# yahoo0742/COSNet

Measured on AMD Instinct MI355X. Metric: frame-pairs/sec (fwd+bwd) at 473x473 RGBD, higher is better.
Workload: dtype bf16; 1 GPU; RGBDSegmentation_RAA train step (fwd+loss+bwd+SGD), 473x473, batch 4 pairs/GPU; model=RGBDSegmentation_RAA(Bottleneck,[3,4,23,3],[3,4,6,3],1), global_batch=4, parallelism=dp1

## Files before the change

cosnet_amd/_native.py:

```python
import ctypes
import os

import torch

_HERE = os.path.dirname(os.path.abspath(__file__))
LIB_PATH = os.environ.get("COSNET_HIP_LIB") or os.path.join(_HERE, "_lib", "libcosnet_hip.so")

DT_F32 = 0
DT_BF16 = 1

_P = ctypes.c_void_p
_I = ctypes.c_int
_L = ctypes.c_longlong
_F = ctypes.c_float
_S = ctypes.c_size_t

_SIGS = {
    "cn_conv_fwd": (_I, [_I, _P, _L, _I, _I, _I, _I, _P, _I, _I, _I, _I, _I, _I, _P, _P, _L, _I, _I, _P]),
    "cn_conv_fwd_ws": (_I, [_I, _P, _L, _I, _I, _I, _I, _P, _I, _I, _I, _I, _I, _I, _P, _P, _L, _I, _I,
                            _P, _S, _P]),
    "cn_conv_fwd_workspace_floats": (_S, [_I, _I, _I, _I]),
    "cn_conv_dgrad": (_I, [_I, _P, _L, _I, _I, _I, _I, _P, _I, _I, _I, _I, _I, _I, _P, _L, _I, _I, _I, _P]),
    "cn_conv_wgrad_workspace_floats": (_S, [_I, _I, _I, _I, _I, _I, _I, _I]),
    "cn_conv_wgrad": (_I, [_I, _P, _L, _I, _I, _I, _I, _P, _L, _I, _I, _I, _I, _I, _I, _I, _I, _P, _P, _P]),
# ... 31 lines not shown
                             _P, _L, _P, _L, _P, _P]),
    "cn_bn_apply_ex": (_I, [_I, _P, _L, _I, _I, _I, _P, _P, _P, _P, _P, _L, _P, _L, _P, _P, _P, _P, _I, _P,
                            _P, _L, _P, _L, _P, _P, _L, _P]),
    "cn_bn_apply_q8": (_I, [_I, _P, _L, _I, _I, _I, _P, _P, _P, _P, _P, _L, _P, _L, _P, _P, _P, _P, _I, _P,
                            _P, _L, _P, _L, _P, _P]),
    "cn_fp8_quant_static": (_I, [_I, _I, _P, _L, _I, _I, _P, _L, _P, _P]),
    "cn_bcast_rows_u8": (_I, [_P, _I, _I, _I, _P, _L, _P]),
    "cn_bn_set_tuning": (_I, [_I, _I]),
    "cn_bn_bwd": (_I, [_I, _P, _L, _P, _L, _P, _L, _I, _I, _P, _P, _P, _P, _I, _P, _P, _P, _P, _P, _L, _P, _L, _P, _P]),
    "cn_coatt_workspace_floats": (_S, [_I, _I, _I]),
    "cn_coatt_softmax": (_I, [_I, _P, _I, _I, _I, _P, _P, _P, _P]),
    "cn_coatt_dscore": (_I, [_I, _P, _P, _P, _P, _P, _P, _I, _I, _I, _P, _P]),
    "cn_coatt_fused_fwd": (_I, [_P, _L, _P, _L, _P, _L, _I, _I, _I, _P, _P, _L, _P]),
    "cn_coatt_fused_fwd_ws": (_I, [_P, _L, _P, _L, _P, _L, _I, _I, _I, _P, _P, _L, _P, _S, _P]),
    "cn_coatt_fused_workspace_bytes": (_S, [_I, _I, _I]),
    "cn_coatt_fused_fwd_idx": (_I, [_P, _L, _P, _L, _P, _L, _P, _P, _I, _I, _I, _P, _P, _L, _P, _S, _P]),
    "cn_gate_cat_idx": (_I, [_I, _P, _L, _P, _L, _P, _I, _I, _I, _P, _P, _P, _L, _P]),
    "cn_mean_groups": (_I, [_P, _I, _I, _I, _P, _P]),
    "cn_coatt_f8_workspace_bytes": (_S, [_I, _I]),
    "cn_coatt_f8_fwd": (_I, [_P, _L, _P, _L, _P, _L, _I, _I, _I, _P, _P, _L, _P, _P, _P, _S, _P]),
    "cn_coatt_f8_train_workspace_bytes": (_S, [_I, _I]),
    "cn_coatt_f8_train_fwd": (_I, [_P, _L, _P, _L, _P, _L, _I, _I, _I, _P, _P, _L, _P, _P, _P, _P, _P, _L, _P, _S, _P]),
    "cn_coatt_f8_bank_bytes": (_S, [_I, _I]),
    "cn_coatt_f8_bank_build": (_I, [_P, _L, _P, _L, _I, _I, _I, _P, _S, _P]),
    "cn_coatt_f8_fwd_idx": (_I, [_P, _P, _I, _P, _P, _I, _I, _I, _P, _P, _L, _P]),
    "cn_coatt_flash_fwd": (_I, [_P, _L, _P, _L, _P, _L, _I, _I, _I, _P, _P, _L, _P, _P, _P]),
    "cn_coatt_flash_fwd_ws": (_I, [_P, _L, _P, _L, _P, _L, _I, _I, _I, _P, _P, _L, _P, _P, _P, _S, _P]),
    "cn_coatt_flash_pv": (_I, [_P, _L, _P, _L, _P, _L, _P, _I, _I, _I, _P, _L, _I, _P]),
    "cn_coatt_flash_dvat": (_I, [_P, _L, _P, _L, _P, _L, _P, _L, _P, _L, _P, _P, _P, _P, _I, _I, _I, _P,
                                 _L, _I, _P]),
    "cn_coatt_flash_dvat_ws": (_I, [_P, _L, _P, _L, _P, _L, _P, _L, _P, _L, _P, _P, _P, _P, _I, _I, _I, _P,
                                    _L, _I, _P, _S, _P]),
    "cn_coatt_flash_bwd_workspace_bytes": (_S, [_I, _I]),
    "cn_coatt_flash_pv_ws": (_I, [_P, _L, _P, _L, _P, _L, _P, _I, _I, _I, _P, _L, _I, _P, _S, _P]),
    "cn_rowdot_seg": (_I, [_I, _P, _L, _P, _L, _I, _I, _I, _I, _P, _P]),
    "cn_nchw_to_nhwc": (_I, [_I, _P, _I, _I, _I, _I, _I, _P, _P]),
    "cn_weight_prep": (_I, [_I, _P, _I, _I, _I, _I, _P, _P, _P]),
    "cn_maxpool_fwd": (_I, [_I, _P, _I, _I, _I, _I, _I, _I, _I, _I, _I, _P, _P, _P]),
    "cn_maxpool_bwd": (_I, [_I, _P, _P, _I, _I, _I, _I, _I, _I, _I, _I, _I, _P, _P]),
    "cn_avgpool": (_I, [_I, _P, _L, _I, _I, _I, _F, _P, _P, _P]),
    "cn_avgpool_workspace_floats": (_S, [_I, _I, _I, _I]),
    "cn_bcast_rows": (_I, [_I, _P, _I, _I, _I, _F, _P, _L, _I, _P]),
    "cn_gate_fwd": (_I, [_I, _P, _L, _I, _I, _P, _P, _P, _L, _P, _P]),
    "cn_gate_bwd": (_I, [_I, _P, _L, _P, _L, _P, _I, _I, _P, _I, _P, _L, _P, _P, _P, _P]),
    "cn_colpart_workspace_floats": (_S, [_I, _I]),
    "cn_mean_rows": (_I, [_P, _I, _I, _P, _P]),
    "cn_sum_rows": (_I, [_P, _I, _I, _P, _P]),
    "cn_scale_dev": (_I, [_P, _L, _P, _P, _P]),
    "cn_scale": (_I, [_P, _L, _F, _P]),
    "cn_soft_iou": (_I, [_P, _P, _I, _L, _P, _P, _P, _P]),
    "cn_frame_resize": (_I, [_I, _P, _I, _L, _L, _L, _I, _I, _I, _I, _P, _P, _I, _I, _I, _I, _P]),
    "cn_gemm_force_config": (_I, [_I]),
    "cn_gemm_ws_mode": (_I, [_I]),
    "cn_gemm_ws_launches": (_S, []),
    "cn_gemm_set_wgrad_target": (_I, [_I]),
    "cn_coatt_force_variant": (_I, [_I]),
    "cn_head_fwd": (_I, [_I, _P, _L, _P, _L, _I, _I, _I, _P, _P, _P, _L, _P, _P]),
    "cn_head_bwd": (_I, [_I, _P, _L, _P, _I, _I, _I, _P, _P, _L, _P, _P, _P, _P]),
    "cn_upsample_sigmoid": (_I, [_P, _I, _I, _I, _I, _I, _I, _P, _P]),
    "cn_upsample_sigmoid_bwd": (_I, [_P, _P, _I, _I, _I, _I, _I, _I, _P, _P]),
    "cn_count_ge": (_I, [_P, _L, _F, _P, _P]),
    "cn_loss_workspace_floats": (_S, [_L]),
    "cn_bce_l1": (_I, [_P, _P, _L, _F, _F, _P, _P, _P, _P]),
    "cn_bce_l1_devcount": (_I, [_P, _P, _L, _P, ctypes.c_double, _F, _P, _P, _P, _P]),
    "cn_sgd": (_I, [_P, _I, _P, _F, _F, _P]),
    "cn_rowdot": (_I, [_I, _P, _L, _P, _L, _I, _I, _P, _P]),
    "cn_colsum": (_I, [_I, _P, _L, _I, _I, _P, _P, _P]),
    "cn_cast2d": (_I, [_I, _I, _P, _L, _I, _I, _P, _L, _I, _P]),
    "cn_build_source_hash": (ctypes.c_char_p, []),
    "cn_build_experimental": (_I, []),
    "cn_conv_wgrad_fp8_workspace_floats": (_S, [_I, _I, _I, _I, _I, _I, _I, _I]),
    "cn_conv_wgrad_fp8": (_I, [_I, _P, _L, _I, _I, _I, _I, _P, _L, _I, _I, _I, _I, _I, _I, _I, _I,
                               _P, _P, _P, _P, _S, _P]),
}

_lib = None


class NativeError(RuntimeError):
    pass


def load():
    global _lib
    if _lib is not None:
        return _lib
    if not os.path.exists(LIB_PATH):
        raise NativeError("libcosnet_hip.so not built (%s); run __graft_entry__.build()" % LIB_PATH)
    lib = ctypes.CDLL(LIB_PATH, mode=ctypes.RTLD_GLOBAL)
    for name, (res, args) in _SIGS.items():
        if os.environ.get("COSNET_HIP_LIB") and not hasattr(lib, name):
            continue
        fn = getattr(lib, name)
        fn.restype = res
        fn.argtypes = args
    _lib = lib
    return lib


HASHED_SOURCES = ["gemm.hip", "gemm_ws.hip", "conv.hip", "bn.hip", "ew.hip", "coatt.hip", "coatt_fused.hip",
                  "coatt_q48.hip", "coatt_flash.hip", "coatt_f8.hip", "fp8.hip", "frames.hip", "eval.hip",
                  "common.h", "gemm.h", "gemm_dev.h", "coatt_fused.h", "../../include/cosnet_hip.h"]


def source_hash():
    import hashlib
# ... 50 lines not shown
```

cosnet_amd/csrc/gemm.hip:

```cpp
#include "common.h"
#include "gemm.h"
#include "gemm_dev.h"
#include "../../include/cosnet_hip.h"

#include <type_traits>

namespace {

template <class T> struct Frag;
template <> struct Frag<bf16> { typedef bf16x8 type; };
template <> struct Frag<float> { typedef f32x4 type; };

__device__ __forceinline__ int mc_swz(int k, int granules_per_row) {
  int h = (k & 3) | (((k >> 3) & 1) << 2);
  return (granules_per_row >= 32 ? h : (h & 3)) << 2;
}

__device__ __forceinline__ int mc_swz8(int k) { return (k & 7) ^ ((k >> 5) & 1); }

__device__ __attribute__((aligned(16))) unsigned g_zero16[4];

__device__ __forceinline__ void glds16(const void* src, char* lds_wave_base) {
  __builtin_amdgcn_global_load_lds((const __attribute__((address_space(1))) void*)src,
                                   (__attribute__((address_space(3))) void*)lds_wave_base, 16, 0, 0);
}

template <class T, int ROWS, int KIND, int NT> struct Loader {
  static constexpr int VEC = VecOf<T>::N;
  static constexpr int BK = 8 * VEC;
  static constexpr int NCH = ROWS * 8 / NT;
  static constexpr int RSTEP = NT / 8;
  static_assert(NCH >= 1 && NCH * NT == ROWS * 8, "tile rows must fill whole chunk rounds");
  static constexpr bool MC = (KIND == L_MC_DENSE || KIND == L_MC_CONV);
  static constexpr bool BUF = (KIND == L_KC_DENSE || KIND == L_KC_CONV || KIND == L_MC_DENSE);
  static constexpr int CPR = ROWS / VEC;
  static constexpr int KROW_STEP = NT / CPR;
  static constexpr int RB = ROWS * (int)sizeof(T);
  static constexpr unsigned SZ = sizeof(T);
  static_assert(!(MC && sizeof(T) == 1) || CPR == 8, "fp8 MC tiles are 128 columns wide (mc_swz8)");

  long long ld;
  int klim;
  int kbeg;
  int kcol;
  bool ok[NCH];
  __amdgpu_buffer_rsrc_t rsrc;
  unsigned voff[NCH];
  int img[NCH], by[NCH], bx[NCH];
  int ctap;
  const T* base;
  const T* ptr[NCH];
  int ry[NCH], sx[NCH], cic[NCH];
  int pim[NCH], poy[NCH], pox[NCH], pp[NCH];
  int ax, ay, aim;
  ConvGeom g;

  __device__ __forceinline__ void init(const T* b, long long ld_, int lim, int klim_,
// ... 103 lines not shown
      }
    } else if constexpr (KIND == L_MC_DENSE) {
      const unsigned soff = (unsigned)(k0 - kbeg) * (unsigned)ld * SZ;
      if (!tail) {
#pragma unroll
        for (int i = 0; i < NCH; ++i) blds16(rsrc, voff[i], soff, wbase + i * NT * 16);
      } else {
        const int kr0 = k0 + tid / CPR;
#pragma unroll
        for (int i = 0; i < NCH; ++i)
          blds16(rsrc, kr0 + KROW_STEP * i < klim ? voff[i] : BUF_OOB, soff, wbase + i * NT * 16);
      }
    } else if constexpr (KIND == L_KC_CONV_G) {
      const void* zp = (const void*)g_zero16;
      const int k = k0 + kcol;
      const bool kok = k < klim;
      int tap, cc;
      fdivmod(kok ? k : 0, g.div_C, tap, cc);
      if (tap != ctap) {
        int r, ss;
        fdivmod(tap, g.div_KW, r, ss);
        const int oy = r * g.step_y, ox = ss * g.step_x;
#pragma unroll
        for (int i = 0; i < NCH; ++i) {
          const int y = by[i] + oy, x = bx[i] + ox;
          const bool v = img[i] >= 0 && (unsigned)y < (unsigned)g.H && (unsigned)x < (unsigned)g.W;
          ok[i] = v;
          const unsigned pix = v ? (unsigned)((img[i] * g.H + y) * g.W + x) : 0u;
          ptr[i] = base + (unsigned long long)pix * (unsigned)ld;
        }
        ctap = tap;
      }
#pragma unroll
      for (int i = 0; i < NCH; ++i)
        glds16((ok[i] && kok) ? (const void*)(ptr[i] + cc) : zp, wbase + i * NT * 16);
    } else {
      const void* zp = (const void*)g_zero16;
#pragma unroll
      for (int i = 0; i < NCH; ++i) {
        const int y = poy[i] * g.st + ry[i], x = pox[i] * g.st + sx[i];
        const bool v = ok[i] && pp[i] < klim && (unsigned)y < (unsigned)g.H && (unsigned)x < (unsigned)g.W;
        const unsigned pix = (unsigned)((pim[i] * g.H + y) * g.W + x);
        const T* src = base + ((unsigned long long)pix * (unsigned)ld + (unsigned)cic[i]);
        glds16(v ? (const void*)src : zp, wbase + i * NT * 16);
        pp[i] += BK;
        pox[i] += ax;
        poy[i] += ay;
        pim[i] += aim;
        if (pox[i] >= g.OW) { pox[i] -= g.OW; poy[i] += 1; }
        if (poy[i] >= g.OH) { poy[i] -= g.OH; pim[i] += 1; }
      }
    }
  }
};

template <int ROWS, bool MC>
__device__ __forceinline__ bf16x8 read_frag_bf16(const char* lds, int rowbase, int p, int lane) {
  int g = lane >> 4;
  if (!MC) {
    int row = rowbase + (lane & 15);
    int c = 4 * p + g;
    return *(const bf16x8*)(lds + row * 128 + ((c ^ (row & 7)) << 4));
  } else {
    constexpr int RB = ROWS * 2;
    int q = (lane & 15) >> 2, pp = lane & 3;
    int gm = (rowbase >> 2) + pp;
    int k1 = 32 * p + 8 * g + q, k2 = k1 + 4;
    const char* a1 = lds + k1 * RB + ((gm ^ mc_swz(k1, RB / 8)) << 3);
    const char* a2 = lds + k2 * RB + ((gm ^ mc_swz(k2, RB / 8)) << 3);
    s16x4 lo = __builtin_amdgcn_ds_read_tr16_b64_v4i16(LDS_PTR(s16x4, a1));
    s16x4 hi = __builtin_amdgcn_ds_read_tr16_b64_v4i16(LDS_PTR(s16x4, a2));
    typedef __attribute__((ext_vector_type(8))) short s16x8;
    s16x8 r = __builtin_shufflevector(lo, hi, 0, 1, 2, 3, 4, 5, 6, 7);
    return __builtin_bit_cast(bf16x8, r);
  }
}

__device__ __forceinline__ i32x8 read_frag_f8(const char* lds, int rowbase, int lane) {
  const int row = rowbase + (lane & 15), g = lane >> 4;
  const u32x4 lo = *(const u32x4*)(lds + row * 128 + (((2 * g) ^ (row & 7)) << 4));
  const u32x4 hi = *(const u32x4*)(lds + row * 128 + (((2 * g + 1) ^ (row & 7)) << 4));
  i32x8 r;
  r[0] = lo.x; r[1] = lo.y; r[2] = lo.z; r[3] = lo.w; r[4] = hi.x; r[5] = hi.y; r[6] = hi.z; r[7] = hi.w;
  return r;
}

typedef __attribute__((ext_vector_type(2))) int i32x2;
__device__ __forceinline__ i32x8 read_frag_f8_mc(const char* lds, int colbase, int lane) {
  const int i = lane & 15, g = lane >> 4, q = i >> 1, pp = i & 1;
  const int cb = colbase >> 4;
  i32x8 r;
#pragma unroll
  for (int j = 0; j < 4; ++j) {
    const int k = 32 * g + 8 * j + q;
    const char* a = lds + k * 128 + ((cb ^ mc_swz8(k)) << 4) + 8 * pp;
    const i32x2 v = __builtin_amdgcn_ds_read_tr8_b64_v2i32(LDS_PTR(i32x2, a));
    r[2 * j] = v.x;
    r[2 * j + 1] = v.y;
  }
  return r;
}

template <int ROWS>
__device__ __forceinline__ f32x4 read_frag_f32_kc(const char* lds, int rowbase, int p, int lane) {
  int row = rowbase + (lane & 15);
  int c = 4 * p + (lane >> 4);
  return *(const f32x4*)(lds + row * 128 + ((c ^ (row & 7)) << 4));
}
template <int ROWS>
__device__ __forceinline__ float read_frag_f32_mc(const char* lds, int rowbase, int p, int j, int lane) {
  int k = 16 * p + 4 * (lane >> 4) + j;
  int col = rowbase + (lane & 15);
  return *(const float*)(lds + k * (ROWS * 4) + col * 4);
}

template <class CT> __device__ __forceinline__ void store_c(CT* c, float v, int mode);
template <> __device__ __forceinline__ void store_c<float>(float* c, float v, int mode) {
  if (mode == 1) atomicAdd(c, v);
  else if (mode == 2) *c += v;
  else *c = v;
}
template <> __device__ __forceinline__ void store_c<bf16>(bf16* c, float v, int mode) {
  if (mode == 2) v += (float)*c;
  *c = (bf16)v;
}

}

template <int G>
__device__ __forceinline__ void wait_tiles(int n) {
  if (n <= 0) asm volatile("s_waitcnt vmcnt(0)" ::: "memory");
  else if (n == 1) asm volatile("s_waitcnt vmcnt(%0)" :: "n"(G) : "memory");
  else if (n == 2) asm volatile("s_waitcnt vmcnt(%0)" :: "n"(2 * G) : "memory");
  else asm volatile("s_waitcnt vmcnt(%0)" :: "n"(3 * G) : "memory");
}

#ifndef CN_GEMM_GROUP_M
#define CN_GEMM_GROUP_M 8
#endif
#ifndef CN_GEMM_PRIO
#define CN_GEMM_PRIO 0
#endif
#ifndef CN_GEMM_ZREMAP
#define CN_GEMM_ZREMAP 1
#endif

template <class T, class CT, int BM, int BN, int WM, int WN, int S, int LA, int LB, int EPI = 0, int PP = 0>
__global__ __launch_bounds__(WM * WN * 64, (EPI && sizeof(T) == 2 && BM * BN <= 128 * 128 && S == 2) ? 4 : 1) void gemm_kernel(GemmArgs p) {
  constexpr int NT = WM * WN * 64;
  constexpr int VEC = VecOf<T>::N;
  constexpr int BK = 8 * VEC;
  constexpr int ABYTES = BM * 128, BBYTES = BN * 128;
  constexpr int STAGE = ABYTES + BBYTES;
  constexpr int TM = BM / WM, TN = BN / WN;
  constexpr int RM = TM / 16, RN = TN / 16;
  constexpr bool AMC = (LA == L_MC_DENSE || LA == L_MC_CONV);
  constexpr bool BMC = (LB == L_MC_DENSE || LB == L_MC_CONV);
  typedef Loader<T, BM, LA, NT> LdA;
  typedef Loader<T, BN, LB, NT> LdB;
  constexpr int G = LdA::NCH + LdB::NCH;
  static_assert(S >= 2 && S <= 4, "2..4 stages");
  __shared__ __attribute__((aligned(16))) char smem[S * STAGE];

  const int tid = threadIdx.x, lane = tid & 63, wave = tid >> 6;
  const int wm = wave / WN, wn = wave % WN;
  int tm, tn, bz;
  {
    const int nwg = gridDim.x * gridDim.y;
#if CN_GEMM_ZREMAP
    const int all = nwg * gridDim.z;
    const int orig = blockIdx.x + blockIdx.y * gridDim.x + blockIdx.z * nwg;
#else
    const int all = nwg;
    const int orig = blockIdx.x + blockIdx.y * gridDim.x;
#endif
    int glin = orig;
    if (all >= 16) {
      const int xcd = orig & 7, q = all >> 3, r = all & 7;
      glin = (xcd < r ? xcd * (q + 1) : r * (q + 1) + (xcd - r) * q) + (orig >> 3);
    }
#if CN_GEMM_ZREMAP
    bz = glin / nwg;
#else
    bz = blockIdx.z;
#endif
    const int lin = glin - (glin / nwg) * nwg;
#if CN_GEMM_GROUP_M > 0
    {
      const int gm = CN_GEMM_GROUP_M;
      const int per = gm * gridDim.y;
      const int grp = lin / per, first = grp * gm;
      const int gsz = min((int)gridDim.x - first, gm);
      const int r = lin - grp * per;
      tm = first + r % gsz;
      tn = r / gsz;
    }
#else
    tm = lin % gridDim.x;
    tn = lin / gridDim.x;
#endif
// ... 52 lines not shown
  static_assert(IT * RPP == HR, "epilogue rows per pass must be a multiple of the row stride");
  constexpr int smode = EPI == 3 ? 0 : EPI;
  constexpr bool PFC = EPI == 3;
  constexpr int PQ = (int)sizeof(CT) / 2;
  static_assert(!PFC || sizeof(CT) == 2, "EPI 3: bf16 C");
  const int c0t = (tid % GPR) * 8;
  CT* Cb = (p.ngroup ? (CT*)p.grp.C[batch] : (CT*)p.C + (long long)batch * p.c_bs) +
           (p.c_mode == 3 ? (long long)split * p.slab : 0);
  u32x4 xnx[(smode == 2 || PFC) ? IT * PQ : 1];
  const __amdgpu_buffer_rsrc_t crs = buf_rsrc(Cb + (long long)m0 * p.ldc);
  auto epi_fetch = [&](int pass) {
#pragma unroll
    for (int it = 0; it < IT; ++it) {
      const int row = m0 + pass * HR + tid / GPR + it * RPP;
      const int col = n0 + c0t;
      if constexpr (smode == 2) {
        const bool ok = row < p.M && col + 8 <= p.N;
        const u32x4* src = (const u32x4*)((const CT*)p.br_x + (long long)(ok ? row : m0) * p.br_ldx + (ok ? col : 0));
#pragma unroll
        for (int q = 0; q < PQ; ++q) xnx[it * PQ + q] = src[q];
      } else if constexpr (PFC) {
        const CT* dst = Cb + (long long)row * p.ldc + col;
        const bool ok = row < p.M && col + 8 <= p.N && ((uintptr_t)dst % 16 == 0);
        xnx[it] = ok ? *(const u32x4*)dst : u32x4{0u, 0u, 0u, 0u};
      }
    }
  };
  constexpr bool EARLY = PFC || (smode == 2 && S >= 3 && BM * BN <= 128 * 128);
  float bk1[8], bsf[8], bmu[8];
  auto epi_affine = [&]() {
#pragma unroll
    for (int e = 0; e < 8; ++e) {
      const int c = n0 + c0t + e;
      const bool in = c < p.N;
      const float g = in ? (p.br_gamma ? p.br_gamma[c] : 1.f) : 0.f;
      const float b = in ? (p.br_beta ? p.br_beta[c] : 0.f) : 0.f;
      const float is = in ? p.br_invstd[c] : 0.f;
      bmu[e] = in ? p.br_mean[c] : 0.f;
      bk1[e] = g * is;
      bsf[e] = b - bmu[e] * bk1[e];
    }
  };
  if constexpr (EARLY) {
    if constexpr (smode == 2) epi_affine();
    epi_fetch(0);
  }

  f32x4 acc[RM][RN];
#pragma unroll
  for (int i = 0; i < RM; ++i)
#pragma unroll
    for (int j = 0; j < RN; ++j) acc[i][j] = (f32x4){0.f, 0.f, 0.f, 0.f};

#pragma unroll
  for (int s = 0; s < S - 1; ++s) {
    if (s < nt) {
      la.issue(kbeg + s * BK, smem + s * STAGE, tid);
      lb.issue(kbeg + s * BK, smem + s * STAGE + ABYTES, tid);
    }
  }
  wait_tiles<G>(min(nt - 1, S - 2));
  raw_barrier();

#if CN_GEMM_PRIO == 2
  if (__builtin_amdgcn_readfirstlane(tid) >= NT / 2) __builtin_amdgcn_s_setprio(1);
#endif
  auto mma_tile = [&](const char* As, const char* Bs) {
    if constexpr (sizeof(T) == 1 && (AMC || BMC)) {
      return;
    } else if constexpr (sizeof(T) == 1) {
      i32x8 af[RM], bfr[RN];
#pragma unroll
      for (int i = 0; i < RM; ++i) af[i] = read_frag_f8(As, wm * TM + i * 16, lane);
#pragma unroll
      for (int j = 0; j < RN; ++j) bfr[j] = read_frag_f8(Bs, wn * TN + j * 16, lane);
#pragma unroll
      for (int i = 0; i < RM; ++i)
#pragma unroll
        for (int j = 0; j < RN; ++j)
          acc[i][j] = __builtin_amdgcn_mfma_scale_f32_16x16x128_f8f6f4(
              af[i], bfr[j], acc[i][j], std::is_same<T, f8e5m2>::value ? 1 : 0, 0, 0, 127, 0, 127);
      return;
    }
#pragma unroll
    for (int pc = 0; pc < 2; ++pc) {
      if constexpr (sizeof(T) == 2) {
        bf16x8 af[RM], bfr[RN];
#pragma unroll
        for (int i = 0; i < RM; ++i) af[i] = read_frag_bf16<BM, AMC>(As, wm * TM + i * 16, pc, lane);
#pragma unroll
        for (int j = 0; j < RN; ++j) bfr[j] = read_frag_bf16<BN, BMC>(Bs, wn * TN + j * 16, pc, lane);
#if CN_GEMM_PRIO == 1
        __builtin_amdgcn_s_setprio(1);
#endif
#pragma unroll
        for (int i = 0; i < RM; ++i)
#pragma unroll
          for (int j = 0; j < RN; ++j)
            acc[i][j] = __builtin_amdgcn_mfma_f32_16x16x32_bf16(af[i], bfr[j], acc[i][j], 0, 0, 0);
#if CN_GEMM_PRIO == 1
        __builtin_amdgcn_s_setprio(0);
#endif
      } else if constexpr (sizeof(T) == 4) {
        f32x4 af[RM], bfr[RN];
        if (!AMC) {
#pragma unroll
          for (int i = 0; i < RM; ++i) af[i] = read_frag_f32_kc<BM>(As, wm * TM + i * 16, pc, lane);
        } else {
#pragma unroll
          for (int i = 0; i < RM; ++i)
#pragma unroll
            for (int j = 0; j < 4; ++j) af[i][j] = read_frag_f32_mc<BM>(As, wm * TM + i * 16, pc, j, lane);
        }
        if (!BMC) {
#pragma unroll
// ... 19 lines not shown
    constexpr int STG = decltype(stg_c)::value;
    constexpr int NXT = (STG + S - 1) % S;
    const char* As = smem + STG * STAGE;
    const char* Bs = As + ABYTES;
    if constexpr (sizeof(T) == 1 && (AMC || BMC)) {
      i32x8 af[RM], bfr[RN];
#pragma unroll
      for (int i = 0; i < RM; ++i)
        af[i] = AMC ? read_frag_f8_mc(As, wm * TM + i * 16, lane) : read_frag_f8(As, wm * TM + i * 16, lane);
#pragma unroll
      for (int j = 0; j < RN; ++j)
        bfr[j] = BMC ? read_frag_f8_mc(Bs, wn * TN + j * 16, lane) : read_frag_f8(Bs, wn * TN + j * 16, lane);
      if (kt + S - 1 < nt) {
        la.issue(kbeg + (kt + S - 1) * BK, smem + NXT * STAGE, tid);
        lb.issue(kbeg + (kt + S - 1) * BK, smem + NXT * STAGE + ABYTES, tid);
      }
#pragma unroll
      for (int i = 0; i < RM; ++i)
#pragma unroll
        for (int j = 0; j < RN; ++j)
          acc[i][j] = __builtin_amdgcn_mfma_scale_f32_16x16x128_f8f6f4(
              af[i], bfr[j], acc[i][j], std::is_same<T, f8e5m2>::value ? 1 : 0, 0, 0, 127, 0, 127);
    } else if constexpr (sizeof(T) == 2 && (AMC || BMC) && (RM + RN) <= 8) {
      bf16x8 af[2][RM], bfr[2][RN];
#pragma unroll
      for (int pc = 0; pc < 2; ++pc) {
#pragma unroll
        for (int i = 0; i < RM; ++i) af[pc][i] = read_frag_bf16<BM, AMC>(As, wm * TM + i * 16, pc, lane);
#pragma unroll
        for (int j = 0; j < RN; ++j) bfr[pc][j] = read_frag_bf16<BN, BMC>(Bs, wn * TN + j * 16, pc, lane);
      }
      if (kt + S - 1 < nt) {
        la.issue(kbeg + (kt + S - 1) * BK, smem + NXT * STAGE, tid);
        lb.issue(kbeg + (kt + S - 1) * BK, smem + NXT * STAGE + ABYTES, tid);
      }
#pragma unroll
      for (int pc = 0; pc < 2; ++pc)
#pragma unroll
        for (int i = 0; i < RM; ++i)
#pragma unroll
          for (int j = 0; j < RN; ++j)
            acc[i][j] = __builtin_amdgcn_mfma_f32_16x16x32_bf16(af[pc][i], bfr[pc][j], acc[i][j], 0, 0, 0);
    } else {
      if (kt + S - 1 < nt) {
        la.issue(kbeg + (kt + S - 1) * BK, smem + NXT * STAGE, tid);
        lb.issue(kbeg + (kt + S - 1) * BK, smem + NXT * STAGE + ABYTES, tid);
      }
      mma_tile(As, Bs);
    }
    wait_tiles<G>(min(nt - 1, kt + S - 1) - (kt + 1));
    raw_barrier();
  };
  constexpr bool PPK = PP == 1 && sizeof(T) == 2 && !AMC && !BMC && WM * WN == 8;
  if constexpr (PPK) {
    const bool g1 = __builtin_amdgcn_readfirstlane(wave) >= 4;
    auto phase_mma = [&](const bf16x8 (&af)[RM], const bf16x8 (&bfr)[RN]) {
      __builtin_amdgcn_sched_barrier(0);
      raw_barrier();
      __builtin_amdgcn_s_setprio(1);
#pragma unroll
      for (int i = 0; i < RM; ++i)
#pragma unroll
        for (int j = 0; j < RN; ++j)
          acc[i][j] = __builtin_amdgcn_mfma_f32_16x16x32_bf16(af[i], bfr[j], acc[i][j], 0, 0, 0);
      __builtin_amdgcn_s_setprio(0);
      __builtin_amdgcn_sched_barrier(0);
      raw_barrier();
    };
    auto refill = [&](int kt, int nxt) {
      la.issue(kbeg + (kt + S - 1) * BK, smem + nxt * STAGE, tid);
      lb.issue(kbeg + (kt + S - 1) * BK, smem + nxt * STAGE + ABYTES, tid);
    };
    auto kstep_pp = [&](int kt, auto stg_c) {
      constexpr int STG = decltype(stg_c)::value;
      constexpr int NXT = (STG + S - 1) % S;
      const char* As = smem + STG * STAGE;
      const char* Bs = As + ABYTES;
      {
        bf16x8 af[RM], bfr[RN];
#pragma unroll
        for (int i = 0; i < RM; ++i) af[i] = read_frag_bf16<BM, false>(As, wm * TM + i * 16, 0, lane);
#pragma unroll
        for (int j = 0; j < RN; ++j) bfr[j] = read_frag_bf16<BN, false>(Bs, wn * TN + j * 16, 0, lane);
        if (S == 2 && kt + S - 1 < nt) refill(kt, NXT);
        phase_mma(af, bfr);
      }
      {
        bf16x8 af[RM], bfr[RN];
#pragma unroll
        for (int i = 0; i < RM; ++i) af[i] = read_frag_bf16<BM, false>(As, wm * TM + i * 16, 1, lane);
#pragma unroll
        for (int j = 0; j < RN; ++j) bfr[j] = read_frag_bf16<BN, false>(Bs, wn * TN + j * 16, 1, lane);
        if (S > 2 && kt + S - 1 < nt) refill(kt, NXT);
        wait_tiles<G>(min(nt - 1, kt + S - 1) - (kt + 1));
        if constexpr (S == 2) asm volatile("s_waitcnt lgkmcnt(0)" ::: "memory");
        phase_mma(af, bfr);
      }
    };
    if (g1) raw_barrier();
    for (int kt = 0; kt < nt; kt += S) {
      kstep_pp(kt, std::integral_constant<int, 0>{});
      if (kt + 1 < nt) kstep_pp(kt + 1, std::integral_constant<int, 1>{});
      if constexpr (S > 2) { if (kt + 2 < nt) kstep_pp(kt + 2, std::integral_constant<int, (S > 2 ? 2 : 0)>{}); }
      if constexpr (S > 3) { if (kt + 3 < nt) kstep_pp(kt + 3, std::integral_constant<int, (S > 3 ? 3 : 0)>{}); }
    }
    if (!g1) raw_barrier();
  } else {
// ... 201 lines not shown
    }
  }
}

struct TileCfg { int bm, bn, wm, wn, s, pp; };
static constexpr TileCfg kCfg[] = {
    {128, 64, 2, 2, 2},
    {128, 128, 2, 2, 2},
    {128, 128, 2, 2, 3},
    {256, 128, 4, 2, 3},
    {128, 256, 2, 4, 3},
    {256, 256, 2, 4, 2},
    {128, 64, 2, 2, 4},
    {128, 128, 2, 2, 4},
    {256, 128, 4, 2, 2},
    {128, 256, 2, 4, 2},
    {256, 256, 4, 2, 2},
    {128, 128, 4, 2, 2},
    {128, 64, 4, 2, 2},
    {128, 128, 4, 2, 3},
    {128, 128, 4, 2, 4},
    {256, 128, 4, 2, 3},
    {128, 64, 4, 2, 4},
    {64, 128, 2, 4, 2},
    {256, 128, 4, 2, 3, 1},
    {128, 256, 2, 4, 3, 1},
    {256, 256, 2, 4, 2, 1},
};
constexpr int kNumCfg = sizeof(kCfg) / sizeof(kCfg[0]);
static int g_force_cfg = -1;

static long long cfg_blocks(int c, const GemmArgs& a, int batch) {
  return (long long)((a.M + kCfg[c].bm - 1) / kCfg[c].bm) * ((a.N + kCfg[c].bn - 1) / kCfg[c].bn) *
         batch * a.nsplit;
}

static long long tiles_of(int c, int M, int N) {
  return (long long)((M + kCfg[c].bm - 1) / kCfg[c].bm) * ((N + kCfg[c].bn - 1) / kCfg[c].bn);
}
static int heuristic_cfg(int M, int N, int K, int bz) {
  if (N <= 64) return 12;
  if (N >= 512 && K >= 2048 && tiles_of(10, M, N) * bz >= 200) return 20;
  if (tiles_of(11, M, N) * bz <= 256 && K >= 512) return 13;
  if (N >= 1024 && K <= 512 && tiles_of(10, M, N) * bz >= 200) return 10;
  return 11;
}

static int pick_cfg(const GemmArgs& a, int batch) {
  if (g_force_cfg >= 0 && g_force_cfg < kNumCfg) return g_force_cfg;
  if (a.cfg >= 0 && a.cfg < kNumCfg) return a.cfg;
  return heuristic_cfg(a.M, a.N, a.K, batch * a.nsplit);
}

template <class T, class CT, int C, int LA, int LB, int EPI = 0>
static int launch_c(const GemmArgs& a, int batch, hipStream_t st) {
  constexpr TileCfg c = kCfg[C];
  dim3 grid((a.M + c.bm - 1) / c.bm, (a.N + c.bn - 1) / c.bn, batch * a.nsplit);
  hipLaunchKernelGGL((gemm_kernel<T, CT, c.bm, c.bn, c.wm, c.wn, c.s, LA, LB, EPI, c.pp>), grid,
                     dim3(c.wm * c.wn * 64), 0, st, a);
  CN_CHECK_LAUNCH();
  return 0;
}

template <class T, int LA, int EPI>
static int launch_epi(const GemmArgs& a, int batch, hipStream_t st) {
  if constexpr (sizeof(T) == 4) {
    if (a.N <= 64 || cfg_blocks(1, a, batch) < 384) return launch_c<T, T, 0, LA, L_KC_DENSE, EPI>(a, batch, st);
    return launch_c<T, T, 1, LA, L_KC_DENSE, EPI>(a, batch, st);
  } else {
    switch (pick_cfg(a, batch)) {
      case 10: return launch_c<T, T, 10, LA, L_KC_DENSE, EPI>(a, batch, st);
      case 11: return launch_c<T, T, 11, LA, L_KC_DENSE, EPI>(a, batch, st);
      case 12: return launch_c<T, T, 12, LA, L_KC_DENSE, EPI>(a, batch, st);
      case 13: return launch_c<T, T, 13, LA, L_KC_DENSE, EPI>(a, batch, st);
      case 18: return launch_c<T, T, 18, LA, L_KC_DENSE, EPI>(a, batch, st);
      case 19: return launch_c<T, T, 19, LA, L_KC_DENSE, EPI>(a, batch, st);
      case 20: return launch_c<T, T, 20, LA, L_KC_DENSE, EPI>(a, batch, st);
      default: return CN_ERR_UNSUPPORTED;
    }
  }
}


template <class T, class CT, int LA, int LB>
static int launch_tile(const GemmArgs& a, int batch, hipStream_t st) {
  if constexpr (sizeof(T) == 2 && sizeof(CT) == 2 && (LA == L_KC_DENSE || LA == L_KC_CONV) &&
                LB == L_KC_DENSE) {
    if (a.c_mode == 2 && !a.row_map && !a.ngroup) {
      switch (pick_cfg(a, batch)) {
        case 10: return launch_c<T, CT, 10, LA, LB, 3>(a, batch, st);
        case 11: return launch_c<T, CT, 11, LA, LB, 3>(a, batch, st);
        case 12: return launch_c<T, CT, 12, LA, LB, 3>(a, batch, st);
        case 13: return launch_c<T, CT, 13, LA, LB, 3>(a, batch, st);
        case 20: return launch_c<T, CT, 20, LA, LB, 3>(a, batch, st);
        default: break;
      }
    }
  }
  if constexpr (sizeof(T) == 4) {
    if (a.N <= 64 || cfg_blocks(1, a, batch) < 384) return launch_c<T, CT, 0, LA, LB>(a, batch, st);
    return launch_c<T, CT, 1, LA, LB>(a, batch, st);
  } else {
    switch (pick_cfg(a, batch)) {
      case 0: return launch_c<T, CT, 0, LA, LB>(a, batch, st);
      case 1: return launch_c<T, CT, 1, LA, LB>(a, batch, st);
      case 2: return launch_c<T, CT, 2, LA, LB>(a, batch, st);
      case 3: return launch_c<T, CT, 3, LA, LB>(a, batch, st);
      case 4: return launch_c<T, CT, 4, LA, LB>(a, batch, st);
      case 5: return launch_c<T, CT, 5, LA, LB>(a, batch, st);
      case 6: return launch_c<T, CT, 6, LA, LB>(a, batch, st);
      case 7: return launch_c<T, CT, 7, LA, LB>(a, batch, st);
      case 8: return launch_c<T, CT, 8, LA, LB>(a, batch, st);
      case 9: return launch_c<T, CT, 9, LA, LB>(a, batch, st);
      case 10: return launch_c<T, CT, 10, LA, LB>(a, batch, st);
      case 11: return launch_c<T, CT, 11, LA, LB>(a, batch, st);
      case 13: return launch_c<T, CT, 13, LA, LB>(a, batch, st);
      case 14: return launch_c<T, CT, 14, LA, LB>(a, batch, st);
      case 15: return launch_c<T, CT, 15, LA, LB>(a, batch, st);
      case 16: return launch_c<T, CT, 16, LA, LB>(a, batch, st);
      case 17: return launch_c<T, CT, 17, LA, LB>(a, batch, st);
      case 18: case 19: case 20: {
        constexpr bool kc = LA != L_MC_DENSE && LA != L_MC_CONV && LB != L_MC_DENSE && LB != L_MC_CONV;
        if constexpr (kc) {
          const int c = pick_cfg(a, batch);
          if (c == 18) return launch_c<T, CT, 18, LA, LB>(a, batch, st);
          if (c == 19) return launch_c<T, CT, 19, LA, LB>(a, batch, st);
          return launch_c<T, CT, 20, LA, LB>(a, batch, st);
        } else {
          if (pick_cfg(a, batch) == 20) return launch_c<T, CT, 10, LA, LB>(a, batch, st);
          return launch_c<T, CT, 11, LA, LB>(a, batch, st);
        }
      }
      default: return launch_c<T, CT, 12, LA, LB>(a, batch, st);
    }
  }
}

template <class T, class CT>
static int launch_conv_g(const GemmArgs& a, int batch, hipStream_t st) {
  if constexpr (sizeof(T) == 4) {
    if (a.N <= 64 || cfg_blocks(1, a, batch) < 384) return launch_c<T, CT, 0, L_KC_CONV_G, L_KC_DENSE>(a, batch, st);
    return launch_c<T, CT, 1, L_KC_CONV_G, L_KC_DENSE>(a, batch, st);
  } else {
    const int c = pick_cfg(a, batch);
    if (c == 12) return launch_c<T, CT, 12, L_KC_CONV_G, L_KC_DENSE>(a, batch, st);
    if (c == 13) return launch_c<T, CT, 13, L_KC_CONV_G, L_KC_DENSE>(a, batch, st);
    return launch_c<T, CT, 11, L_KC_CONV_G, L_KC_DENSE>(a, batch, st);
  }
}

template <class T, class CT>
static int launch_kinds(const GemmArgs& a, int la, int lb, int batch, hipStream_t st) {
#define CN_CASE(A_, B_) \
  if (la == A_ && lb == B_) return launch_tile<T, CT, A_, B_>(a, batch, st);
  if (la == L_KC_CONV_G && lb == L_KC_DENSE) return launch_conv_g<T, CT>(a, batch, st);
  CN_CASE(L_KC_DENSE, L_KC_DENSE)
  CN_CASE(L_KC_CONV, L_KC_DENSE)
  CN_CASE(L_KC_DENSE, L_MC_DENSE)
  CN_CASE(L_MC_DENSE, L_MC_DENSE)
  CN_CASE(L_MC_DENSE, L_MC_CONV)
#undef CN_CASE
  return -10;
}

template <class CT, int LA, class T8 = f8e4m3>
static int launch_f8(const GemmArgs& a, int batch, hipStream_t st) {
  const int c = pick_cfg(a, batch);
  if constexpr (sizeof(CT) == 2 && std::is_same<T8, f8e4m3>::value) {
    if (a.st_mode == 1) {
      if (c == 12) return launch_c<T8, CT, 12, LA, L_KC_DENSE, 1>(a, batch, st);
      if (c == 13) return launch_c<T8, CT, 13, LA, L_KC_DENSE, 1>(a, batch, st);
      return launch_c<T8, CT, 11, LA, L_KC_DENSE, 1>(a, batch, st);
    }
  }
  if (a.st_mode) return CN_ERR_UNSUPPORTED;
  if (c == 12) return launch_c<T8, CT, 12, LA, L_KC_DENSE>(a, batch, st);
  if (c == 13) return launch_c<T8, CT, 13, LA, L_KC_DENSE>(a, batch, st);
  return launch_c<T8, CT, 11, LA, L_KC_DENSE>(a, batch, st);
}

// ... 61 lines not shown
    return CN_ERR_UNSUPPORTED;
  }
  if (a.st_mode) {
    if ((batch != 1 && !(a.ngroup == batch && a.st_mode == 1)) || a.nsplit != 1 || a.row_map || a.c_mode ||
        lb != L_KC_DENSE || (la != L_KC_DENSE && la != L_KC_CONV && la != L_KC_CONV_G))
      return CN_ERR_UNSUPPORTED;
#define CN_EPI(T_, M_) \
    return la == L_KC_DENSE ? launch_epi<T_, L_KC_DENSE, M_>(a, batch, st) : \
           la == L_KC_CONV ? launch_epi<T_, L_KC_CONV, M_>(a, batch, st) : launch_epi<T_, L_KC_CONV_G, M_>(a, batch, st)
    if (dtype == DT_BF16) {
      if (a.st_mode == 1) CN_EPI(bf16, 1); else CN_EPI(bf16, 2);
    } else {
      if (a.st_mode == 1) CN_EPI(float, 1); else CN_EPI(float, 2);
    }
#undef CN_EPI
  }
  if (dtype == DT_BF16) {
    return c_f32 ? launch_kinds<bf16, float>(a, la, lb, batch, st)
                 : launch_kinds<bf16, bf16>(a, la, lb, batch, st);
  } else if (dtype == DT_F32) {
    return launch_kinds<float, float>(a, la, lb, batch, st);
  }
  return -11;
}

int cn_gemm_bm(int dtype, int M, int N, int K, int cfg) {
  if (dtype != DT_BF16) return kCfg[1].bm;
  if (g_force_cfg >= 0 && g_force_cfg < kNumCfg) return kCfg[g_force_cfg].bm;
  if (cfg >= 0 && cfg < kNumCfg) return kCfg[cfg].bm;
  return kCfg[heuristic_cfg(M, N, K, 1)].bm;
}

int cn_gemm_pick(int M, int N, int K, int batch_splits) {
  if (g_force_cfg >= 0 && g_force_cfg < kNumCfg) return g_force_cfg;
  return heuristic_cfg(M, N, K, batch_splits);
}

long long cn_gemm_cfg_blocks(int cfg, int M, int N) {
  GemmArgs a = {};
  a.M = M; a.N = N; a.nsplit = 1;
  return cfg_blocks(cfg, a, 1);
}

extern "C" int cn_gemm_force_config(int cfg) {
  if (cfg >= kNumCfg) return -1;
  g_force_cfg = cfg;
  return kNumCfg;
}

extern "C" int cn_gemm_ws_mode(int mode) {
  if (mode < 0 || mode > 3) return -1;
  const int prev = g_ws_mode;
  g_ws_mode = mode;
  return prev;
}

extern "C" size_t cn_gemm_ws_launches(void) { return g_ws_launches; }

template <int G>
__global__ __launch_bounds__(256) void splitk_reduce_k(const float* __restrict__ ws, int nsplit,
                                                       long long slab, long long n4,
                                                       float* __restrict__ out, int accumulate) {
  constexpr int OPB = 256 / G;
  __shared__ f32x4 red[G][OPB];
  const int o = threadIdx.x % OPB, g = threadIdx.x / OPB;
  for (long long base = (long long)blockIdx.x * OPB; base < n4; base += (long long)gridDim.x * OPB) {
    const long long i = base + o;
    f32x4 a = {0.f, 0.f, 0.f, 0.f};
    if (i < n4) {
      int s = g;
      for (; s + 7 * G < nsplit; s += 8 * G) {
        f32x4 v[8];
#pragma unroll
        for (int u = 0; u < 8; ++u) v[u] = *(const f32x4*)(ws + (long long)(s + u * G) * slab + 4 * i);
#pragma unroll
        for (int u = 0; u < 8; ++u) a += v[u];
      }
      for (; s < nsplit; s += G) a += *(const f32x4*)(ws + (long long)s * slab + 4 * i);
    }
    if (G > 1) {
      red[g][o] = a;
      __syncthreads();
      if (g == 0) {
#pragma unroll
        for (int q = 1; q < G; ++q) a += red[q][o];
      }
      __syncthreads();
    }
    if (g == 0 && i < n4) {
      if (accumulate) a += ((const f32x4*)out)[i];
      ((f32x4*)out)[i] = a;
    }
  }
}

int cn_splitk_reduce_impl(const float* ws, int nsplit, long long slab, long long n, float* out,
                          int accumulate, hipStream_t st) {
  if (n % 4 || slab % 4) return -2;
  const long long n4 = n / 4;
  int G = 1;
  while (G < 16 && 2 * G <= nsplit && n4 * G < (512ll << 10)) G *= 2;
  const int opb = 256 / G;
  long long b = (n4 + opb - 1) / opb;
  if (b > 4096) b = 4096;
#define CN_RED(GG) \
  hipLaunchKernelGGL(splitk_reduce_k<GG>, dim3((unsigned)b), dim3(256), 0, st, ws, nsplit, slab, n4, out, accumulate)
// ... 12 lines not shown
```

include/cosnet_hip.h:

```cpp
#ifndef COSNET_HIP_H
#define COSNET_HIP_H
#include <stddef.h>
#include <hip/hip_runtime_api.h>

#ifdef __cplusplus
extern "C" {
#endif

#define CN_ERR_SHAPE (-1)
#define CN_ERR_ALIGN (-2)
#define CN_ERR_UNSUPPORTED (-3)
#define CN_ERR_HIP (-4)


int cn_conv_fwd(int dtype, const void* x, long long ldx, int N, int H, int W, int Cin,
                const void* w, int Cout, int KH, int KW, int stride, int pad, int dil,
                const float* bias, void* y, long long ldy, int OH, int OW, hipStream_t stream);

size_t cn_conv_fwd_workspace_floats(int dtype, int M, int Cout, int K);
int cn_conv_fwd_ws(int dtype, const void* x, long long ldx, int N, int H, int W, int Cin,
                   const void* w, int Cout, int KH, int KW, int stride, int pad, int dil,
                   const float* bias, void* y, long long ldy, int OH, int OW, float* ws,
                   size_t ws_floats, hipStream_t stream);

// ... 195 lines not shown
                const float* gb, void* out, long long ldo, float* mask, hipStream_t stream);
int cn_gate_bwd(int dtype, const void* z, long long ldz, const void* dout, long long lddo,
                const float* mask, int P, int C, const float* g, int through_mask, void* dz,
                long long lddz, float* dg, float* dgb,
                float* ws , hipStream_t stream);
int cn_mean_rows(const float* x, int nrows, int C, float* out, hipStream_t stream);
int cn_mean_groups(const float* x, int ngroups, int n, int C, float* out, hipStream_t stream);
int cn_gate_cat_idx(int dtype, const void* z, long long ldz, const void* vbank, long long ldv,
                    const int* iv, int P, int HW, int C, const float* g, const float* gb, void* out,
                    long long ldo, hipStream_t stream);
int cn_sum_rows(const float* x, int nrows, int C, float* out, hipStream_t stream);
int cn_scale(float* x, long long n, float s, hipStream_t stream);
int cn_scale_dev(const float* x, long long n, const float* s, float* out, hipStream_t stream);
int cn_soft_iou(const float* x, const unsigned char* gt, int nframes, long long hw,
                unsigned char* mask, double* iou, long long* counts, hipStream_t stream);
size_t cn_colpart_workspace_floats(int P, int C);
int cn_head_fwd(int dtype, const void* a, long long lda, const void* b, long long ldb, int P,
                int C, int relu, const float* w, const float* bias, void* zout, long long ldz,
                float* logit, hipStream_t stream);
int cn_head_bwd(int dtype, const void* z, long long ldz, const float* dlogit, int P, int C,
                int relu, const float* w, void* dz, long long lddz, float* dw, float* db,
                float* ws , hipStream_t stream);
int cn_upsample_sigmoid(const float* in, int N, int h, int w, int H, int W, int apply_sigmoid,
                        float* out, hipStream_t stream);
int cn_upsample_sigmoid_bwd(const float* dout, const float* out, int N, int h, int w, int H,
                            int W, int apply_sigmoid, float* din, hipStream_t stream);
int cn_count_ge(const float* gt, long long n, float thr, unsigned long long* cnt,
                hipStream_t stream);
size_t cn_loss_workspace_floats(long long n);
int cn_bce_l1(const float* pred, const float* gt, long long n, float weight, float l1w, float* ws,
              float* loss, float* dpred, hipStream_t stream);
int cn_bce_l1_devcount(const float* pred, const float* gt, long long n, const long long* pos_count,
                       double total, float l1w, float* ws, float* loss, float* dpred,
                       hipStream_t stream);
int cn_sgd(const void* tensors, int nt, const float* lrs, float wd, float momentum,
           hipStream_t stream);
int cn_rowdot(int dtype, const void* a, long long lda, const void* b, long long ldb, int P, int C,
              float* out, hipStream_t stream);
int cn_rowdot_seg(int dtype, const void* a, long long lda, const void* b, long long ldb, int P, int C,
                  int seg, int seg_ld, float* out, hipStream_t stream);
int cn_colsum(int dtype, const void* x, long long ld, int P, int C, float* out,
              float* ws , hipStream_t stream);
int cn_cast2d(int dtype_in, int dtype_out, const void* x, long long ldx, int P, int C, void* y,
              long long ldy, int accumulate, hipStream_t stream);
int cn_frame_resize(int src_u8, const void* src, int C, long long plane_stride, long long row_stride,
                    long long col_stride, int y0, int x0, int h, int w, const float* mean,
                    float* dst, int H, int W, int mode, int flip, hipStream_t stream);

const char* cn_build_source_hash(void);
int cn_build_experimental(void);

int cn_gemm_force_config(int cfg);
int cn_gemm_ws_mode(int mode);
size_t cn_gemm_ws_launches(void);
int cn_gemm_set_wgrad_target(int blocks);
int cn_coatt_force_variant(int v);

#ifdef __cplusplus
}
#endif
#endif
```

Before: 135.9 frame-pairs/s.

## Add deep-K software-pipelined main loop for 256x256 bf16 GEMM config

Adds a new main loop for tile configuration 20 (256x256, 8 waves, 2 stages) on k-contiguous bf16 operands. Each K-tile is split into four MFMA quadrants, with loads for the next one or two tiles issued between quadrants, fine-grained vmcnt waits and priority raises, and wave-group staggered barriers. The aim is to hide global-to-LDS latency and LDS fragment reads behind matrix-core work. It is enabled by default for selected epilogue and loader classes and can be switched off through an environment variable and an API knob. The hand-tuned waitcnt accounting could be fragile if the load counts per round change.

```diff
diff --git a/cosnet_amd/_native.py b/cosnet_amd/_native.py
--- a/cosnet_amd/_native.py
+++ b/cosnet_amd/_native.py
@@ -107,6 +107,7 @@
     "cn_frame_resize": (_I, [_I, _P, _I, _L, _L, _L, _I, _I, _I, _I, _P, _P, _I, _I, _I, _I, _P]),
     "cn_gemm_force_config": (_I, [_I]),
     "cn_gemm_ws_mode": (_I, [_I]),
+    "cn_gemm_deep_loop": (_I, [_I]),
     "cn_gemm_ws_launches": (_S, []),
     "cn_gemm_set_wgrad_target": (_I, [_I]),
     "cn_coatt_force_variant": (_I, [_I]),
diff --git a/cosnet_amd/csrc/gemm.hip b/cosnet_amd/csrc/gemm.hip
--- a/cosnet_amd/csrc/gemm.hip
+++ b/cosnet_amd/csrc/gemm.hip
@@ -3,6 +3,7 @@
 #include "gemm_dev.h"
 #include "../../include/cosnet_hip.h"
 
+#include <cstdlib>
 #include <type_traits>
 
 namespace {
@@ -212,6 +213,46 @@
       }
     }
   }
+
+  template <int I0, int I1>
+  __device__ __forceinline__ void issue_rounds(int k0, char* lds, int tid) {
+    static_assert(KIND == L_KC_DENSE || KIND == L_KC_CONV, "buffer-descriptor k-contiguous loaders");
+    static_assert(NCH == 4 && I0 >= 0 && I0 < I1 && I1 < NCH, "two distinct rounds of four");
+    char* wbase = lds + __builtin_amdgcn_readfirstlane((tid & ~63) * 16);
+    const bool tail = k0 + BK > klim;
+    unsigned soff;
+    if constexpr (KIND == L_KC_DENSE) {
+      soff = (unsigned)k0 * SZ;
+    } else {
+      const int tap = __builtin_amdgcn_readfirstlane(fdiv(k0, g.div_C));
+      if (tap != ctap) {
+        int r, ss;
+        fdivmod(tap, g.div_KW, r, ss);
+        const int oy = r * g.step_y, ox = ss * g.step_x;
+#pragma unroll
+        for (int i = 0; i < NCH; ++i) {
+          const int y = by[i] + oy, x = bx[i] + ox;
+          const bool v = img[i] >= 0 && (unsigned)y < (unsigned)g.H && (unsigned)x < (unsigned)g.W;
+          const unsigned pix = (unsigned)((img[i] * g.H + y) * g.W + x);
+          voff[i] = v ? (pix * (unsigned)ld + (unsigned)kcol) * SZ : BUF_OOB;
+        }
+        ctap = tap;
+      }
+      soff = (unsigned)(k0 - tap * g.C) * SZ;
+    }
+    if (!tail) {
+      blds16(rsrc, voff[I0], soff, wbase + I0 * NT * 16);
+      blds16(rsrc, voff[I1], soff, wbase + I1 * NT * 16);
+    } else {
+      const bool kok = k0 + kcol < klim;
+      blds16(rsrc, kok ? voff[I0] : BUF_OOB, soff, wbase + I0 * NT * 16);
+      blds16(rsrc, kok ? voff[I1] : BUF_OOB, soff, wbase + I1 * NT * 16);
+    }
+  }
+  template <int H>
+  __device__ __forceinline__ void issue_half(int k0, char* lds, int tid) {
+    issue_rounds<2 * H, 2 * H + 1>(k0, lds, tid);
+  }
 };
 
 template <int ROWS, bool MC>
@@ -305,7 +346,7 @@
 #define CN_GEMM_ZREMAP 1
 #endif
 
-template <class T, class CT, int BM, int BN, int WM, int WN, int S, int LA, int LB, int EPI = 0, int PP = 0>
+template <class T, class CT, int BM, int BN, int WM, int WN, int S, int LA, int LB, int EPI = 0, int PP = 0, int DL = 0>
 __global__ __launch_bounds__(WM * WN * 64, (EPI && sizeof(T) == 2 && BM * BN <= 128 * 128 && S == 2) ? 4 : 1) void gemm_kernel(GemmArgs p) {
   constexpr int NT = WM * WN * 64;
   constexpr int VEC = VecOf<T>::N;
@@ -464,6 +505,10 @@
 #pragma unroll
     for (int j = 0; j < RN; ++j) acc[i][j] = (f32x4){0.f, 0.f, 0.f, 0.f};
 
+  constexpr bool DEEP = DL == 1 && PP == 1 && sizeof(T) == 2 && BM == 256 && BN == 256 && WM == 2 && WN == 4 &&
+                        S == 2 && (LA == L_KC_DENSE || LA == L_KC_CONV) && LB == L_KC_DENSE;
+  static_assert(DL == 0 || DEEP, "the deep-K loop is configuration 20 on k-contiguous bf16 operands");
+  if constexpr (!DEEP) {
 #pragma unroll
   for (int s = 0; s < S - 1; ++s) {
     if (s < nt) {
@@ -473,6 +518,7 @@
   }
   wait_tiles<G>(min(nt - 1, S - 2));
   raw_barrier();
+  }
 
 #if CN_GEMM_PRIO == 2
   if (__builtin_amdgcn_readfirstlane(tid) >= NT / 2) __builtin_amdgcn_s_setprio(1);
@@ -598,7 +644,106 @@
     raw_barrier();
   };
   constexpr bool PPK = PP == 1 && sizeof(T) == 2 && !AMC && !BMC && WM * WN == 8;
-  if constexpr (PPK) {
+  if constexpr (DEEP) {
+    const bool g1 = __builtin_amdgcn_readfirstlane(wave) >= 4;
+    auto part = [&](int t, auto u_c) {
+      constexpr int U = decltype(u_c)::value;
+      char* stg = smem + (t & 1) * STAGE;
+      const int k0 = kbeg + t * BK;
+      if constexpr (U == 0) la.template issue_rounds<0, 2>(k0, stg, tid);
+      else if constexpr (U == 1) lb.template issue_half<0>(k0, stg + ABYTES, tid);
+      else if constexpr (U == 2) lb.template issue_half<1>(k0, stg + ABYTES, tid);
+      else la.template issue_rounds<1, 3>(k0, stg, tid);
+    };
+    auto quad = [&](const bf16x8 (&af)[4][2], const bf16x8 (&bfr)[2][2], auto ih_c, auto jh_c) {
+      constexpr int I0 = 4 * decltype(ih_c)::value, J0 = 2 * decltype(jh_c)::value;
+      __builtin_amdgcn_sched_barrier(0);
+      raw_barrier();
+      asm volatile("s_waitcnt lgkmcnt(0)" ::: "memory");
+      __builtin_amdgcn_sched_barrier(0);
+      __builtin_amdgcn_s_setprio(1);
+#pragma unroll
+      for (int pc = 0; pc < 2; ++pc)
+#pragma unroll
+        for (int i = 0; i < 4; ++i)
+#pragma unroll
+          for (int j = 0; j < 2; ++j)
+            acc[I0 + i][J0 + j] =
+                __builtin_amdgcn_mfma_f32_16x16x32_bf16(af[i][pc], bfr[j][pc], acc[I0 + i][J0 + j], 0, 0, 0);
+      __builtin_amdgcn_s_setprio(0);
+      __builtin_amdgcn_sched_barrier(0);
+      raw_barrier();
+    };
+    using c0 = std::integral_constant<int, 0>;
+    using c1 = std::integral_constant<int, 1>;
+    using c2 = std::integral_constant<int, 2>;
+    using c3 = std::integral_constant<int, 3>;
+    auto ktile = [&](int t, auto buf_c) {
+      constexpr int BUF = decltype(buf_c)::value;
+      const char* As = smem + BUF * STAGE;
+      const char* Bs = As + ABYTES;
+      const int rem = nt - 1 - t;
+      bf16x8 a0[4][2], a1[4][2], b0[2][2], b1[2][2];
+#pragma unroll
+      for (int j = 0; j < 2; ++j)
+#pragma unroll
+        for (int pc = 0; pc < 2; ++pc) b0[j][pc] = read_frag_bf16<BN, false>(Bs, wn * TN + j * 16, pc, lane);
+      __builtin_amdgcn_sched_barrier(0);
+#pragma unroll
+      for (int i = 0; i < 4; ++i)
+#pragma unroll
+        for (int pc = 0; pc < 2; ++pc) a0[i][pc] = read_frag_bf16<BM, false>(As, wm * TM + i * 16, pc, lane);
+      __builtin_amdgcn_sched_barrier(0);
+      if (rem >= 1) part(t + 1, c2{});
+      quad(a0, b0, c0{}, c0{});
+#pragma unroll
+      for (int j = 0; j < 2; ++j)
+#pragma unroll
+        for (int pc = 0; pc < 2; ++pc) b1[j][pc] = read_frag_bf16<BN, false>(Bs, wn * TN + (2 + j) * 16, pc, lane);
+      __builtin_amdgcn_sched_barrier(0);
+      if (rem >= 1) {
+        part(t + 1, c3{});
+        asm volatile("s_waitcnt vmcnt(8)" ::: "memory");
+      } else {
+        asm volatile("s_waitcnt vmcnt(0)" ::: "memory");
+      }
+      quad(a0, b1, c0{}, c1{});
+#pragma unroll
+      for (int i = 0; i < 4; ++i)
+#pragma unroll
+        for (int pc = 0; pc < 2; ++pc) a1[i][pc] = read_frag_bf16<BM, false>(As, wm * TM + (4 + i) * 16, pc, lane);
+      __builtin_amdgcn_sched_barrier(0);
+      if (rem >= 2) part(t + 2, c0{});
+      quad(a1, b1, c1{}, c1{});
+      if (rem >= 2) {
+        part(t + 2, c1{});
+        asm volatile("s_waitcnt vmcnt(6)" ::: "memory");
+      } else if (rem == 1) {
+        asm volatile("s_waitcnt vmcnt(2)" ::: "memory");
+      }
+      quad(a1, b0, c1{}, c0{});
+    };
+    if (nt >= 1) {
+      part(0, c0{});
+      part(0, c1{});
+      part(0, c2{});
+      part(0, c3{});
+      if (nt >= 2) {
+        part(1, c0{});
+        part(1, c1{});
+        asm volatile("s_waitcnt vmcnt(6)" ::: "memory");
+      } else {
+        asm volatile("s_waitcnt vmcnt(2)" ::: "memory");
+      }
+    }
+    raw_barrier();
+    if (g1) raw_barrier();
+    for (int t = 0; t < nt; t += 2) {
+      ktile(t, c0{});
+      if (t + 1 < nt) ktile(t + 1, c1{});
+    }
+    if (!g1) raw_barrier();
+  } else if constexpr (PPK) {
     const bool g1 = __builtin_amdgcn_readfirstlane(wave) >= 4;
     auto phase_mma = [&](const bf16x8 (&af)[RM], const bf16x8 (&bfr)[RN]) {
       __builtin_amdgcn_sched_barrier(0);
@@ -906,14 +1051,41 @@
   return heuristic_cfg(a.M, a.N, a.K, batch * a.nsplit);
 }
 
-template <class T, class CT, int C, int LA, int LB, int EPI = 0>
+template <class T, class CT, int C, int LA, int LB, int EPI = 0, int DL = 0>
 static int launch_c(const GemmArgs& a, int batch, hipStream_t st) {
   constexpr TileCfg c = kCfg[C];
   dim3 grid((a.M + c.bm - 1) / c.bm, (a.N + c.bn - 1) / c.bn, batch * a.nsplit);
-  hipLaunchKernelGGL((gemm_kernel<T, CT, c.bm, c.bn, c.wm, c.wn, c.s, LA, LB, EPI, c.pp>), grid,
+  hipLaunchKernelGGL((gemm_kernel<T, CT, c.bm, c.bn, c.wm, c.wn, c.s, LA, LB, EPI, c.pp, DL>), grid,
                      dim3(c.wm * c.wn * 64), 0, st, a);
   CN_CHECK_LAUNCH();
   return 0;
+}
+
+#ifndef CN_GEMM_DEEP_LOOP_DEFAULT
+#define CN_GEMM_DEEP_LOOP_DEFAULT 1
+#endif
+static int deep_loop_env() {
+  const char* e = getenv("CN_GEMM_DEEP_LOOP");
+  if (e && e[0] >= '0' && e[0] <= '2' && !e[1]) return e[0] - '0';
+  return CN_GEMM_DEEP_LOOP_DEFAULT;
+}
+static int g_deep_loop = deep_loop_env();
+
+template <int LA, int EPI, class CT>
+static constexpr bool deep_class() {
+  if (EPI == 1) return true;
+  if (EPI == 3) return LA == L_KC_DENSE;
+  return LA == L_KC_CONV && sizeof(CT) == 4;
+}
+
+template <class T, class CT, int LA, int LB, int EPI = 0>
+static int launch_c20(const GemmArgs& a, int batch, hipStream_t st) {
+  if constexpr (sizeof(T) == 2 && (LA == L_KC_DENSE || LA == L_KC_CONV) && LB == L_KC_DENSE && EPI != 2 &&
+                !(LA == L_KC_CONV && EPI == 3)) {
+    if (g_deep_loop == 2 || (g_deep_loop == 1 && deep_class<LA, EPI, CT>()))
+      return launch_c<T, CT, 20, LA, LB, EPI, 1>(a, batch, st);
+  }
+  return launch_c<T, CT, 20, LA, LB, EPI>(a, batch, st);
 }
 
 template <class T, int LA, int EPI>
@@ -929,7 +1101,7 @@
       case 13: return launch_c<T, T, 13, LA, L_KC_DENSE, EPI>(a, batch, st);
       case 18: return launch_c<T, T, 18, LA, L_KC_DENSE, EPI>(a, batch, st);
       case 19: return launch_c<T, T, 19, LA, L_KC_DENSE, EPI>(a, batch, st);
-      case 20: return launch_c<T, T, 20, LA, L_KC_DENSE, EPI>(a, batch, st);
+      case 20: return launch_c20<T, T, LA, L_KC_DENSE, EPI>(a, batch, st);
       default: return CN_ERR_UNSUPPORTED;
     }
   }
@@ -946,7 +1118,7 @@
         case 11: return launch_c<T, CT, 11, LA, LB, 3>(a, batch, st);
         case 12: return launch_c<T, CT, 12, LA, LB, 3>(a, batch, st);
         case 13: return launch_c<T, CT, 13, LA, LB, 3>(a, batch, st);
-        case 20: return launch_c<T, CT, 20, LA, LB, 3>(a, batch, st);
+        case 20: return launch_c20<T, CT, LA, LB, 3>(a, batch, st);
         default: break;
       }
     }
@@ -979,7 +1151,7 @@
           const int c = pick_cfg(a, batch);
           if (c == 18) return launch_c<T, CT, 18, LA, LB>(a, batch, st);
           if (c == 19) return launch_c<T, CT, 19, LA, LB>(a, batch, st);
-          return launch_c<T, CT, 20, LA, LB>(a, batch, st);
+          return launch_c20<T, CT, LA, LB>(a, batch, st);
         } else {
           if (pick_cfg(a, batch) == 20) return launch_c<T, CT, 10, LA, LB>(a, batch, st);
           return launch_c<T, CT, 11, LA, LB>(a, batch, st);
@@ -1147,6 +1319,14 @@
   if (mode < 0 || mode > 3) return -1;
   const int prev = g_ws_mode;
   g_ws_mode = mode;
+  return prev;
+}
+
+extern "C" int cn_gemm_deep_loop(int mode) {
+  if (mode == -1) return g_deep_loop;
+  if (mode < 0 || mode > 2) return -1;
+  const int prev = g_deep_loop;
+  g_deep_loop = mode;
   return prev;
 }
 
diff --git a/include/cosnet_hip.h b/include/cosnet_hip.h
--- a/include/cosnet_hip.h
+++ b/include/cosnet_hip.h
@@ -271,6 +271,7 @@
 
 int cn_gemm_force_config(int cfg);
 int cn_gemm_ws_mode(int mode);
+int cn_gemm_deep_loop(int mode);
 size_t cn_gemm_ws_launches(void);
 int cn_gemm_set_wgrad_target(int blocks);
 int cn_coatt_force_variant(int v);
```

After: 137.1 frame-pairs/s, median of 6. About the same (+0.9%).
